# alexkeroro86/SampleNeRFRO

Measured on AMD Instinct MI355X. Metric: rays/sec (train step), higher is better.
Workload: dtype f16x3/fp32-acc

## Files before the change

include/rnerf.h:

```cpp
#ifndef RNERF_H_
#define RNERF_H_

#include <stddef.h>
#include <stdint.h>

#ifdef __cplusplus
extern "C" {
#endif

#define RNERF_VERSION 4

enum rnerf_status {
  RNERF_OK = 0,
  RNERF_ERR_ARG = -1,
  RNERF_ERR_HIP = -2,
  RNERF_ERR_UNSUPPORTED = -3
};

enum rnerf_precision {
  RNERF_PREC_F32 = 0,
  RNERF_PREC_F16X3 = 1,
  RNERF_PREC_BF16X3 = 2,
  RNERF_PREC_F16 = 3,
  RNERF_PREC_BF16 = 4,
// ... 29 lines not shown
const char* rnerf_last_error(void);
int rnerf_version(void);
int rnerf_device_cus(void);

int rnerf_grid_prefilter(const float* src, float* dst, float* tmp, const int32_t dims[3], int ksize, double ksigma,
                         void* stream);

int rnerf_grid_build_table(const float* grid, float* table, const rnerf_grid* g, void* stream);

int rnerf_grid_query(const float* table, const rnerf_grid* g, const float* pts, int64_t n, float* out, int32_t* idx,
                     void* stream);

int rnerf_march(const float* table, const rnerf_grid* g, const float* origins, const float* viewdirs, int32_t B,
                double near, double far, int32_t num_nodes, float* path_pd, float* path_dr, float* path_ior,
                int32_t* vox, void* stream);

size_t rnerf_nerfmlp_packed_bytes(int precision);
int rnerf_nerfmlp_pack(const float* params, int precision, void* packed, void* stream);

int rnerf_nerfmlp_forward(const void* packed, int precision, const float* rows_pd, const float* rows_dr,
                          const int32_t* node_of_sample, int32_t S, int32_t B, float* out_raw, int32_t max_workgroups, void* stream);

int rnerf_bkgd_forward(const float* params, const float* dirs, int32_t dir_stride, int64_t n, double rgb_padding,
                       float* out_rgb, void* stream);

int rnerf_composite(const float* raw, const float* rows_pd, const float* rows_dr, const int32_t* node_of_sample,
                    int32_t S, int32_t B, const float* bkgd, int white_bkgd, double rgb_padding, double sigma_bias,
                    float* rgb, float* dist, float* acc, float* trans, float* trans_bkgd, float* weights,
                    float* alpha, int mask_mode, const double* bbox, void* stream);

// ... 117 lines not shown
  int32_t randomized;
  int32_t use_random_choice;
  int32_t bg_patch_size;
  double bg_weight, bg_smooth_weight, annealed_alpha;
  double frozen_sq;
  int64_t frozen_count;
  void* aux_stream;
  void* grads_stream;
} rnerf_train_cfg;
typedef struct rnerf_prefetch {
  const float* origins;
  const float* viewdirs;
  float* path_pd;
  float* path_dr;
  void* side_stream;
} rnerf_prefetch;
size_t rnerf_train_workspace_bytes(const rnerf_model* m, const rnerf_train_cfg* c, int32_t B);
int rnerf_train_forward_backward(const rnerf_model* m, const rnerf_train_cfg* c, const float* theta, const float* origins, const float* viewdirs,
                                 const float* pixels, const float* env_dirs, int32_t B, const uint32_t* keys4, const int32_t* jitter_override,
                                 const float* u_override, int32_t u_per_ray, const float* path_pd, const float* path_dr, float* grads,
                                 void* workspace, int32_t max_workgroups, const rnerf_prefetch* next, void* stream);

#define RNERF_ADAM_SCRATCH_FLOATS 3076
typedef struct rnerf_adam_cfg {
  double lr_init, lr_final, lr_delay_mult;
  int64_t max_steps, lr_delay_steps;
  double b1, b2, eps;
  double weight_decay_mult, grad_max_val, grad_max_norm;
  int64_t n_all;
  double lr_override;
// ... 91 lines not shown
```

samplenerfro_amd/_lib.py:

```python
from __future__ import annotations

import ctypes as C
import os
from typing import Optional

HERE = os.path.dirname(os.path.abspath(__file__))
LIB_PATH = os.path.join(HERE, "lib", "librnerf.so")

PREC_F32, PREC_F16X3, PREC_BF16X3, PREC_F16, PREC_BF16, PREC_F16X2, PREC_F16F8 = 0, 1, 2, 3, 4, 5, 6
PRECISIONS = {"f32": PREC_F32, "f16x3": PREC_F16X3, "bf16x3": PREC_BF16X3, "f16": PREC_F16, "bf16": PREC_BF16, "f16x2": PREC_F16X2, "f16f8": PREC_F16F8}
BWD_BF16, BWD_F16, BWD_F16X2 = 0, 1, 2
BWD_F16X3 = BWD_F16X2
BWD_F16X3_LO8 = 4
BACKWARDS = {"f16x3": BWD_F16X3, "f16x3lo8": BWD_F16X3_LO8, "f16": BWD_F16, "bf16": BWD_BF16, "f32": BWD_F16X3, "tf32": BWD_F16}
BACKWARD_NAMES = {BWD_F16X3: "f16x3", BWD_F16X3_LO8: "f16x3lo8", BWD_F16: "f16", BWD_BF16: "bf16"}
TWO_PLANE_BACKWARDS = (BWD_F16X3, BWD_F16X3_LO8)
ABI_VERSION = 4
NERFMLP_PARAMS = 595844
BKGDMLP_PARAMS = 56963
SO3MLP_PARAMS = 65411
LPIPS_WEIGHT_FLOATS = 2470848


class RnerfError(RuntimeError):
# ... 25 lines not shown

class TrainCfg(C.Structure):
    _fields_ = [("backward", C.c_int32), ("randomized", C.c_int32), ("use_random_choice", C.c_int32), ("bg_patch_size", C.c_int32),
                ("bg_weight", C.c_double), ("bg_smooth_weight", C.c_double), ("annealed_alpha", C.c_double), ("frozen_sq", C.c_double),
                ("frozen_count", C.c_int64), ("aux_stream", C.c_void_p), ("grads_stream", C.c_void_p)]


class AdamCfg(C.Structure):
    _fields_ = [("lr_init", C.c_double), ("lr_final", C.c_double), ("lr_delay_mult", C.c_double), ("max_steps", C.c_int64),
                ("lr_delay_steps", C.c_int64), ("b1", C.c_double), ("b2", C.c_double), ("eps", C.c_double), ("weight_decay_mult", C.c_double),
                ("grad_max_val", C.c_double), ("grad_max_norm", C.c_double), ("n_all", C.c_int64), ("lr_override", C.c_double),
                ("use_lr_override", C.c_int32), ("skip_nonfinite", C.c_int32)]


class Prefetch(C.Structure):
    _fields_ = [("origins", C.c_void_p), ("viewdirs", C.c_void_p), ("path_pd", C.c_void_p), ("path_dr", C.c_void_p), ("side_stream", C.c_void_p)]


LEVEL_FLOATS = 9
ADAM_SCRATCH_FLOATS = 3076
_vp, _i32, _i64, _dbl = C.c_void_p, C.c_int32, C.c_int64, C.c_double
_GP = C.POINTER(Grid)
_MP, _TP, _AP = C.POINTER(Model), C.POINTER(TrainCfg), C.POINTER(AdamCfg)

SIGNATURES = {
    "rnerf_last_error": (C.c_char_p, []),
    "rnerf_version": (C.c_int, []),
    "rnerf_device_cus": (C.c_int, []),
    "rnerf_grid_prefilter": (C.c_int, [_vp, _vp, _vp, C.POINTER(_i32 * 3), C.c_int, _dbl, _vp]),
    "rnerf_grid_table_floats": (C.c_size_t, [_GP]),
    "rnerf_grid_build_table": (C.c_int, [_vp, _vp, _GP, _vp]),
    "rnerf_grid_query": (C.c_int, [_vp, _GP, _vp, _i64, _vp, _vp, _vp]),
    "rnerf_march": (C.c_int, [_vp, _GP, _vp, _vp, _i32, _dbl, _dbl, _i32, _vp, _vp, _vp, _vp, _vp]),
    "rnerf_nerfmlp_packed_bytes": (C.c_size_t, [C.c_int]),
    "rnerf_nerfmlp_pack": (C.c_int, [_vp, C.c_int, _vp, _vp]),
    "rnerf_nerfmlp_forward": (C.c_int, [_vp, C.c_int, _vp, _vp, _vp, _i32, _i32, _vp, _i32, _vp]),
    "rnerf_bkgd_forward": (C.c_int, [_vp, _vp, _i32, _i64, _dbl, _vp, _vp]),
    "rnerf_composite": (C.c_int, [_vp, _vp, _vp, _vp, _i32, _i32, _vp, C.c_int, _dbl, _dbl,
                                  _vp, _vp, _vp, _vp, _vp, _vp, _vp, C.c_int, C.POINTER(C.c_double * 6), _vp]),
    "rnerf_loss_reduce": (C.c_int, [_vp, _vp, _vp, _vp, _vp, _i32, _vp, _vp]),
    "rnerf_env_smooth_sum_floats": (C.c_size_t, [_i32]),
    "rnerf_env_smooth_backward": (C.c_int, [_vp, _i32, _dbl, _vp, _vp, _vp]),
    "rnerf_train_stats": (C.c_int, [_vp, _i32, _i32, _dbl, _vp, _i32, _dbl, _vp, _i64, _dbl, _i64, _vp, _vp]),
    "rnerf_composite_backward": (C.c_int, [_vp, _vp, _vp, _vp, _i32, _i32, _vp, _dbl, _dbl, _vp, _vp, _vp, _vp, _vp, _dbl, _dbl,
                                           _vp, _vp, C.c_int, C.c_int, C.c_int, C.POINTER(C.c_double * 6), _vp]),
    "rnerf_nerfmlp_save_bytes": (C.c_size_t, [_i64, C.c_int]),
    "rnerf_nerfmlp_dy_bytes": (C.c_size_t, [_i64, C.c_int]),
    "rnerf_nerfmlp_bwd_packed_bytes": (C.c_size_t, []),
# ... 120 lines not shown
```

samplenerfro_amd/csrc/march.hip:

```cpp
#include "common.h"

#include <stdlib.h>

namespace rnerf {

struct MarchParams {
  int dx, dy, dz;
  float nmin[3];
  double rcp_nd[3];
  unsigned sa[3], sb[3];
};

constexpr int kMarchAhead = 2;
constexpr int kMarchSets = kMarchAhead + 1;
constexpr int kMarchChunk = kMarchSets <= 4 ? 2 * kMarchSets : kMarchSets;
static_assert(2 * kMarchChunk * 512 <= 12 * 1024, "the ring must fit beside the weight-gradient kernel's LDS (148 KiB)");

__device__ __forceinline__ void march_chunk_barrier() { asm volatile("s_waitcnt lgkmcnt(0)\n\ts_barrier" ::: "memory"); }

template <bool WANT_IOR, bool WANT_VOX, bool BRICKS>
__global__ void __launch_bounds__(128) march_kernel(const float* __restrict__ table, MarchParams g,
                                                    const float* __restrict__ origins, const float* __restrict__ viewdirs,
                                                    int B, float near, float step, int num_nodes,
                                                    float* __restrict__ path_pd, float* __restrict__ path_dr,
                                                    float* __restrict__ path_ior, int* __restrict__ vox, int rays_per_wg) {
  constexpr int C = kMarchChunk;
  __shared__ float2 ring[2][C][64];
  const int lane = threadIdx.x & 63;
  const int wave = __builtin_amdgcn_readfirstlane((int)(threadIdx.x >> 6));
  const int q = lane & 3;
  int r = blockIdx.x * rays_per_wg + ((lane >> 2) & (rays_per_wg - 1));
  if (r >= B) r = B - 1;
  const int qc = q < 3 ? q : 0;
  const int nchunks = (num_nodes + C - 1) / C;
  const size_t node_stride = 4 * (size_t)B;

  if (wave != 0) {
    float* __restrict__ out_pd = path_pd + 4 * (size_t)r + q;
    float* __restrict__ out_dr = path_dr + 4 * (size_t)r + q;
    float rt = near, p_prev = 0.f;
    for (int c = 0; c < nchunks; ++c) {
      march_chunk_barrier();
      const float2* __restrict__ src = &ring[c & 1][0][lane];
#pragma unroll
      for (int s = 0; s < C; ++s) {
        const int k = c * C + s;
        if (k >= num_nodes) break;
        const float2 v = src[s * 64];
        const float p = v.x, d = v.y;
        if (k > 0) rt = fadd(rt, fsqrt(quad_sumsq3(fsub(p_prev, p))));
        p_prev = p;
        const float nrm = fsqrt(fmaxf(quad_sumsq3(d), 1e-6f));
        *out_pd = q < 3 ? p : rt;
        *out_dr = q < 3 ? fdiv(d, nrm) : 0.f;
        out_pd += node_stride; out_dr += node_stride;
      }
    }
    return;
  }

  const float nmin_q = g.nmin[qc];
  const double rcp_q = g.rcp_nd[qc];
  const int dim_q = qc == 0 ? g.dx : (qc == 1 ? g.dy : g.dz);
  const unsigned comp = (q + 1) & 3;
  const char* __restrict__ tabc = (const char*)table;
  const unsigned cofs = comp * 4u;
  const unsigned stride_q = g.sb[qc];
  const unsigned sa_q = g.sa[qc], sb_q = g.sb[qc];
  const int hi_q = dim_q - 1;
  float d = q < 3 ? viewdirs[3 * r + qc] : 0.f;
// ... 59 lines not shown
    d = fadd(d, fmul(step, c));
  };
  static_assert(C % kMarchSets == 0, "a chunk is a whole number of register rotations");
  for (int c = 0, k = 0; c < nchunks; ++c, k += C) {
    float2* slot = &ring[c & 1][0][lane];
#pragma unroll
    for (int u = 0; u < C; ++u) one_step(k + u, cs[u % kMarchSets], cs[(u + kMarchAhead) % kMarchSets], slot + 64 * u);
    march_chunk_barrier();
  }
}

}

using namespace rnerf;

extern "C" int rnerf_march(const float* table, const rnerf_grid* g, const float* origins, const float* viewdirs,
                           int32_t B, double near, double far, int32_t num_nodes, float* path_pd, float* path_dr,
                           float* path_ior, int32_t* vox, void* stream) {
  RNERF_CHECK_ARG(table && g && origins && viewdirs && path_pd && path_dr, "rnerf_march: null pointer");
  RNERF_CHECK_ARG(B > 0 && num_nodes >= 2, "rnerf_march: need B > 0 and num_nodes >= 2");
  RNERF_CHECK_ARG((((uintptr_t)table | (uintptr_t)path_pd | (uintptr_t)path_dr | (uintptr_t)path_ior) & 15) == 0,
                  "rnerf_march: table/path buffers must be 16-byte aligned");
  GridParams gp;
  RNERF_CHECK_ARG(make_grid_params(g, &gp), "rnerf_march: bad grid");
  RNERF_CHECK_ARG(grid_fits_march(gp), "rnerf_march: grid too large for 32-bit byte offsets (needs a table < 4 GiB and 24-bit strides: the row strides in reference order, the brick strides in bricks)");
  MarchParams p;
  p.dx = gp.dx; p.dy = gp.dy; p.dz = gp.dz;
  p.nmin[0] = gp.nminx; p.nmin[1] = gp.nminy; p.nmin[2] = gp.nminz;
  p.rcp_nd[0] = 1.0 / (double)gp.ndx; p.rcp_nd[1] = 1.0 / (double)gp.ndy; p.rcp_nd[2] = 1.0 / (double)gp.ndz;
  for (int i = 0; i < 3; ++i) { p.sa[i] = gp.sa[i]; p.sb[i] = gp.sb[i]; }
  const float stepf = (float)((far - near) / (num_nodes - 1));
  const float nearf = (float)near;
  const int rpw = 16;
  const dim3 block(128), grid((B + rpw - 1) / rpw);
  hipStream_t st = (hipStream_t)stream;
#define LAUNCH2(I, V, K)                                                                                           \
  hipLaunchKernelGGL((march_kernel<I, V, K>), grid, block, 0, st, table, p, origins, viewdirs, B, nearf, stepf, num_nodes, \
                     path_pd, path_dr, path_ior, vox, rpw)
#define LAUNCH(I, V) do { if (gp.layout == RNERF_TABLE_BRICKS) LAUNCH2(I, V, true); else LAUNCH2(I, V, false); } while (0)
  if (path_ior && vox) LAUNCH(true, true);
  else if (path_ior) LAUNCH(true, false);
  else if (vox) LAUNCH(false, true);
  else LAUNCH(false, false);
#undef LAUNCH
#undef LAUNCH2
  RNERF_CHECK_LAUNCH();
  return RNERF_OK;
}
```

samplenerfro_amd/csrc/pipeline.hip:

```cpp
#include "common.h"

#include <math.h>
#include <mutex>
#include <utility>
#include <vector>

namespace rnerf {
static int current_device_cus() {
  static int cache[64] = {0};
  int dev = 0;
  if (hipGetDevice(&dev) != hipSuccess || dev < 0 || dev >= 64) return 256;
  if (cache[dev] == 0) {
    int cus = 0;
    cache[dev] = (hipDeviceGetAttribute(&cus, hipDeviceAttributeMultiprocessorCount, dev) == hipSuccess && cus > 0) ? cus : 256;
  }
  return cache[dev];
}

namespace {
constexpr size_t kPoolCap = 32;
struct EventPool { std::vector<hipEvent_t> free_[64]; };
thread_local EventPool tl_pool;
inline hipError_t pool_get(hipEvent_t* e) {
  int dev = 0;
// ... 521 lines not shown
  if (aux) {
    RNERF_TRY(rnerf_fork(stream, aux));
    void* streams[2] = {t.packed_c, t.packed_f};
    void* dys[2] = {t.dy, t.dy_c};
    const int64_t dy_rows[2] = {(int64_t)(Nf > 0 ? S : Nc) * B, (int64_t)Nc * B};
    RNERF_TRY(nerfmlp_step_zero(prec, streams, Nf > 0 ? 2 : 1, bwd, dys, dy_rows, t.dy_c ? 2 : 1, (hipStream_t)aux));
    pre_zeroed = true;
    RNERF_TRY(nerfmlp_pack_impl(th_c, prec, t.packed_c, false, (hipStream_t)aux, false));
  }
  const int32_t* jitter = jitter_override;
  if (keys4) {
    RNERF_TRY(rnerf_rng_forward(keys4, Nc, m->num_path, c->use_random_choice, t.jitter, t.key_u, stream));
    if (!jitter_override) jitter = t.jitter;
  }
  if (!path_pd) {
    RNERF_TRY(rnerf_march(m->table, &m->grid, origins, viewdirs, B, m->near, m->far, N, f.path_pd, f.path_dr, nullptr, nullptr, stream));
    path_pd = f.path_pd; path_dr = f.path_dr;
  }
  hipLaunchKernelGGL(bkgd_dirs_kernel, dim3((B + M + 255) / 256), dim3(256), 0, st, (const float4*)path_dr, jitter, Nc, B, env_dirs, M, (float4*)f.bk_dirs);
  RNERF_CHECK_LAUNCH();
  RNERF_TRY(rnerf_bkgd_forward_train(th_b, f.bk_dirs, 4, (int64_t)B + M, m->rgb_padding, t.out_all, t.save_bk, stream));
  const float* bkgd = t.out_all;
  const float* rgb_env = t.out_all + (size_t)3 * B;
  if (aux) {
    RNERF_TRY(rnerf_join(stream, aux));
    if (Nf > 0) {
      RNERF_TRY(nerfmlp_pack_impl(th_f, prec, t.packed_f, false, (hipStream_t)aux, false));
      RNERF_TRY(mark_point((hipStream_t)aux, &fine_packed.e));
    }
    RNERF_CHECK_HIP(hipMemsetAsync(grads, 0, (size_t)(n_theta + 8) * sizeof(float), (hipStream_t)aux));
    RNERF_TRY(rnerf_nerfmlp_pack_bwd(th_c, bwd, t.packed_bwd, aux));
// ... 15 lines not shown
    if (!aux) RNERF_TRY(rnerf_nerfmlp_pack(th_f, prec, t.packed_f, stream));
    else { hipEvent_t e = fine_packed.e; fine_packed.e = nullptr; RNERF_TRY(wait_point(st, e)); }
    RNERF_TRY(rnerf_nerfmlp_forward_train(t.packed_f, prec, f.rows_pd, f.rows_dr, nullptr, S, B, f.raw_f, t.save_f, bwd, max_workgroups, stream));
    lf = level_of(t.level_f, B);
    RNERF_TRY(rnerf_composite(f.raw_f, f.rows_pd, f.rows_dr, nullptr, S, B, bkgd, m->white_bkgd, m->rgb_padding, m->sigma_bias, lf.rgb, lf.dist, lf.acc, lf.trans,
                              lf.tb, nullptr, nullptr, level_mask_mode(m), level_mask_box(m), stream));
    if (m->bd_cut == 1) RNERF_TRY(bd_cut_pair(m, f.raw_f, f.rows_pd, f.rows_dr, S, B, bkgd, lf, f.tmp_level, f.tmp_level2, stream));
  }
  RNERF_TRY(rnerf_loss_reduce(Nf > 0 ? lc.rgb : nullptr, lf.rgb, lf.trans, lf.tb, pixels, B, t.sums, stream));
  const double bg_on = (c->bg_weight > 0 && c->annealed_alpha > 0) ? 1.0 : 0.0;
  const double mse_scale = 2.0 / (3.0 * B);
  const double env_on = c->annealed_alpha > 0 ? 1.0 : 0.0;
  if (!aux) RNERF_CHECK_HIP(hipMemsetAsync(grads, 0, (size_t)(n_theta + 8) * sizeof(float), st));
  auto march_next = [&]() -> int {
    RNERF_CHECK_ARG(next->origins && next->viewdirs && next->path_pd && next->path_dr && next->side_stream, "rnerf_train_forward_backward: incomplete rnerf_prefetch");
    RNERF_TRY(rnerf_fork(stream, next->side_stream));
    return rnerf_march(m->table, &m->grid, next->origins, next->viewdirs, B, m->near, m->far, N, next->path_pd, next->path_dr, nullptr, nullptr,
                       next->side_stream);
  };
  if (aux) RNERF_TRY(rnerf_join(stream, aux));
  float* d_first = t.d_all;
  const bool split_levels = levels_side_by_side(m, c, B);
  float* d_raw_c = split_levels ? t.d_raw_c : t.d_raw;
  void* dy_c = split_levels ? t.dy_c : t.dy;
  if (Nf > 0) {
    RNERF_TRY(rnerf_composite_backward(f.raw_f, f.rows_pd, f.rows_dr, nullptr, S, B, bkgd, m->rgb_padding, m->sigma_bias, lf.rgb, pixels, lf.trans, lf.tb, t.sums,
                                       mse_scale, c->bg_weight * bg_on, t.d_raw, d_first, 0, m->white_bkgd, m->bd_cut == 1 ? 1 : level_mask_mode(m), m->bd_cut ? m->bd_cut_bbox : nullptr, stream));
    if (split_levels) {
      RNERF_TRY(rnerf_composite_backward(f.raw_c, path_pd, path_dr, jitter, Nc, B, bkgd, m->rgb_padding, m->sigma_bias, lc.rgb, pixels, nullptr, nullptr, nullptr,
                                         mse_scale, 0.0, d_raw_c, d_first, 1, m->white_bkgd, level_mask_mode(m), level_mask_box(m), stream));
      RNERF_TRY(rnerf_fork(stream, aux));
      if (smooth) RNERF_TRY(rnerf_env_smooth_backward(rgb_env, ps, c->bg_smooth_weight * env_on, t.d_all + (size_t)3 * B, t.env_sum, aux));
      RNERF_TRY(rnerf_bkgd_backward(th_b, t.save_bk, t.d_all, (int64_t)B + M, m->rgb_padding, t.dy_bk, g_b, nullptr, aux));
// ... 181 lines not shown
```

samplenerfro_amd/models.py:

```python
from __future__ import annotations

import ctypes as C
import math
import os
import weakref
from typing import Any, Dict, List, Optional, Sequence, Tuple

import numpy as np
import torch

from . import _lib, ops, prng
from ._lib import Grid, PRECISIONS
from .utils import Rays

NERF_MLP_SHAPES = [(63, 256), (256, 256), (256, 256), (256, 256), (256, 256), (319, 256), (256, 256), (256, 256),
                   (256, 1), (256, 256), (283, 128), (128, 3)]
BKGD_MLP_SHAPES = [(27, 128), (128, 128), (128, 128), (155, 128), (128, 3)]
SO3_MLP_SHAPES = [(60, 128), (128, 128), (128, 128), (188, 128), (128, 3)]


_STREAMS: Dict[Tuple[str, str], "torch.cuda.Stream"] = {}


def shared_stream(device, role: str) -> "torch.cuda.Stream":
# ... 197 lines not shown
            raise NotImplementedError("prefetch_path: the all* march depends on the so3_mlp parameters; call apply() without a handle")
        if self._side is None:
            self._side = shared_stream(self.device, "march")
        self._mlp_wg_limit = max(_lib.load().rnerf_device_cus() - int(reserve_cus), 1) if reserve_cus > 0 else 0
        cur = torch.cuda.current_stream()
        if sync_inputs:
            self._side.wait_stream(cur)
        with torch.cuda.stream(self._side):
            rays.origins.record_stream(self._side); rays.viewdirs.record_stream(self._side)
            pd, dr, ior, _ = ops.march(self.table, self.spec, rays.origins, rays.viewdirs, self.near, self.far,
                                       self.num_samples, want_ior=self.use_online_sparsity)
            ev = torch.cuda.Event()
            ev.record(self._side)
        return PathHandle(pd, dr, ior, ev, rays.origins.shape[0])

    def prefetch_slot(self, rays: Rays):
        if not self.stage.startswith("radiance"):
            raise NotImplementedError("prefetch: the all* march depends on the so3_mlp parameters")
        if self._side is None:
            self._side = shared_stream(self.device, "march")
        o, v = ops._chk(rays.origins, "origins"), ops._chk(rays.viewdirs, "viewdirs")
        B = o.shape[0]
        pd = torch.empty((self.num_samples, B, 4), dtype=torch.float32, device=self.device)
        dr = torch.empty_like(pd)
        for t in (o, v, pd, dr):
            t.record_stream(self._side)
        h = PathHandle(pd, dr, None, torch.cuda.Event(), B)
        h.keep = (o, v)
        return h, _lib.Prefetch(o.data_ptr(), v.data_ptr(), pd.data_ptr(), dr.data_ptr(), self._side.cuda_stream)

    def tail_stream(self) -> torch.cuda.Stream:
        if getattr(self, "_tail", None) is None:
            self._tail = shared_stream(self.device, "tail")
        return self._tail

    def comm_stream(self) -> torch.cuda.Stream:
        return self.tail_stream()

    def release_reserved_cus(self) -> None:
        self._mlp_wg_limit = 0

    def c_model(self, variables=None, precision: Optional[int] = None) -> "_lib.Model":
        prec = self.precision if precision is None else int(precision)
        m = _lib.Model()
# ... 56 lines not shown
        if Nf > 0:
            if u_fine is not None:
                u = ops._chk(u_fine, "u_fine"); per_ray = 1 if u.dim() == 2 else 0
            elif not randomized:
                u = self.make_u(None, B, False)
            else:
                if jitter is not None:
                    key, _ = prng.split(np.asarray(rng_1, np.uint32))
                    u = self.make_u(key, B, True)
                else:
                    u = torch.empty((Nf, B), dtype=torch.float32, device=self.device)
                    _lib.check(lib.rnerf_stratified_u_dev(key_u.data_ptr(), B, Nf, u.data_ptr(), st), "rnerf_stratified_u_dev")
                per_ray = 1
        pd = dr = None
        if path is not None:
            if path.batch != B:
                raise ValueError("path handle was marched for a different batch size")
            cur = torch.cuda.current_stream()
            cur.wait_event(path.event)
            pd, dr = path.pd, path.dr
            pd.record_stream(cur); dr.record_stream(cur)
        ws = self._workspace("fwd", lib.rnerf_forward_workspace_bytes(C.byref(m), B))
        out_c = torch.empty(_lib.LEVEL_FLOATS * B, dtype=torch.float32, device=self.device)
        out_f = torch.empty(_lib.LEVEL_FLOATS * B, dtype=torch.float32, device=self.device) if Nf > 0 else None
        _lib.check(lib.rnerf_forward(C.byref(m), o.data_ptr(), v.data_ptr(), B, jit.data_ptr(), _lib.ptr(u), per_ray, _lib.ptr(pd), _lib.ptr(dr),
                                     out_c.data_ptr(), _lib.ptr(out_f), ws.data_ptr(), int(self._mlp_wg_limit), st), "rnerf_forward")
        return [level_views(t, B) for t in (out_c, out_f) if t is not None]

    def apply(self, variables, *args, method=None, **kwargs):
        if method is not None:
# ... 4 lines not shown
                jitter=None, u_fine: Optional[torch.Tensor] = None, taps: Optional[dict] = None,
                path: Optional["PathHandle"] = None, ctx: Optional[dict] = None,
                noise_c: Optional[torch.Tensor] = None, noise_f: Optional[torch.Tensor] = None):
        origins, viewdirs = rays.origins, rays.viewdirs
        if origins.dim() != 2 or origins.shape[-1] != 3:
            raise ValueError("rays.origins must be [B, 3]")
        B = origins.shape[0]
        noisy = self.noise_std is not None and randomized
        if ctx is None and taps is None and self.whole_path and self.stage.startswith("radiance") and not self.use_online_sparsity and not noisy:
            return self._forward_whole(variables, rng_0, rng_1, rays, randomized, jitter, u_fine, path), 0.0
        Nc, Nf, N = self.num_coarse_samples, self.num_fine_samples, self.num_samples
        key, rng_0 = prng.split(np.asarray(rng_0, np.uint32))
        sparsity = self.use_online_sparsity and (ctx is None or (bool(ctx.get("loss_sp")) and not self.stage.startswith("all")))
        want_ior = sparsity or (taps is not None and not (ctx is not None and self.stage.startswith("all")))
        if path is not None:
            if path.batch != B:
                raise ValueError("path handle was marched for a different batch size")
            cur = torch.cuda.current_stream()
            cur.wait_event(path.event)
            path_pd, path_dr, path_ior = path.pd, path.dr, path.ior
            for t in (path_pd, path_dr, path_ior):
                if t is not None:
                    t.record_stream(cur)
            if want_ior and path_ior is None:
                raise ValueError("path handle lacks the IoR record (prefetch it from a model with the same options)")
        elif self.stage.startswith("all") and ctx is not None:
            rec = ops.march_all_train(self.table, self.spec, self._flat(variables, "so3_mlp", SO3_MLP_SHAPES).detach(), origins, viewdirs,
                                      self.near, self.far, N, annealed_alpha, lazy=True)
            ctx["march_rec"] = rec
            path_pd, path_dr, path_ior = rec["path_pd"], rec["path_dr"], None
# ... 142 lines not shown
        loss_sp = (alpha - coarse_alpha_target).abs().mean()
        next_c, next_f = alpha.mean(), 0.0
        if self.num_fine_samples > 0 and self.use_fine_sparsity:
            alpha = alpha_of("fine_mlp", self.fine_step_size)
            loss_sp = loss_sp + (alpha - fine_alpha_target).abs().mean()
            next_f = alpha.mean()
        return loss_sp, next_c, next_f


def level_views(out: torch.Tensor, B: int):
    return (out[:3 * B].view(B, 3), out[3 * B:4 * B], out[4 * B:5 * B], out[5 * B:6 * B].view(B, 1), out[6 * B:9 * B].view(B, 3))


class PathHandle:

    def __init__(self, pd, dr, ior, event, batch):
        self.pd, self.dr, self.ior, self.event, self.batch = pd, dr, ior, event, batch


def make_variables(flat: Dict[str, torch.Tensor]) -> Dict[str, Any]:
    params: Dict[str, Any] = {"coarse_mlp": flat_to_tree(flat["coarse_mlp"], NERF_MLP_SHAPES),
                              "bkgd_mlp": flat_to_tree(flat["bkgd_mlp"], BKGD_MLP_SHAPES)}
    if "fine_mlp" in flat:
        params["fine_mlp"] = flat_to_tree(flat["fine_mlp"], NERF_MLP_SHAPES)
    if "so3_mlp" in flat:
        params["path_sampler"] = {"scan": {"idx_model": {"so3_mlp": flat_to_tree(flat["so3_mlp"], SO3_MLP_SHAPES)}}}
    return {"params": params, "flat": dict(flat)}


def construct_nerf(key, example_batch, args, ndim, nmin, nmax, grid, precision: str = "f16x3", device=None, eval_precision: Optional[str] = None):
    if args.rgb_activation != "sigmoid" or args.sigma_activation != "softplus" or args.net_activation != "relu":
        raise NotImplementedError("the HIP kernels implement relu / sigmoid / softplus (the reference defaults, rnerf/utils.py:168-175)")
# ... 17 lines not shown
```

samplenerfro_amd/ops.py:

```python
from __future__ import annotations

import ctypes as C
import os
import weakref
from typing import Optional, Tuple

import torch

from . import _lib
from ._lib import Grid, check, current_stream, ptr


def _chk(t: torch.Tensor, name: str, dtype=torch.float32) -> torch.Tensor:
    if not t.is_cuda:
        raise _lib.RnerfError(f"{name}: expected a CUDA (ROCm) tensor; the hot path has no CPU implementation")
    if t.dtype != dtype:
        raise _lib.RnerfError(f"{name}: expected dtype {dtype}, got {t.dtype}")
    return t if t.is_contiguous() else t.contiguous()


_workspaces: dict = {}


def workspace(name: str, *args, device, keep_for: Optional[int] = None) -> torch.Tensor:
# ... 81 lines not shown
def march(table: torch.Tensor, spec: Grid, origins: torch.Tensor, viewdirs: torch.Tensor, near: float, far: float,
          num_nodes: int, want_ior: bool = False, want_vox: bool = False, out=None):
    lib = _lib.load()
    table = _chk(table, "table"); o = _chk(origins, "origins"); d = _chk(viewdirs, "viewdirs")
    B = o.shape[0]
    if out is not None:
        path_pd, path_dr = out
    else:
        path_pd = torch.empty((num_nodes, B, 4), dtype=torch.float32, device=o.device)
        path_dr = torch.empty((num_nodes, B, 4), dtype=torch.float32, device=o.device)
    ior = torch.empty((num_nodes, B, 4), dtype=torch.float32, device=o.device) if want_ior else None
    vox = torch.empty((num_nodes, B, 6), dtype=torch.int32, device=o.device) if want_vox else None
    check(lib.rnerf_march(ptr(table), C.byref(spec), ptr(o), ptr(d), B, float(near), float(far), int(num_nodes),
                          ptr(path_pd), ptr(path_dr), ptr(ior), ptr(vox), current_stream()), "rnerf_march")
    return path_pd, path_dr, ior, vox


def nerfmlp_pack(params_flat: torch.Tensor, precision: int, out: Optional[torch.Tensor] = None) -> torch.Tensor:
    lib = _lib.load()
    p = _chk(params_flat, "params_flat")
    if p.numel() != _lib.NERFMLP_PARAMS:
        raise _lib.RnerfError(f"NerfMLP flat params must have {_lib.NERFMLP_PARAMS} floats, got {p.numel()}")
    nbytes = lib.rnerf_nerfmlp_packed_bytes(int(precision))
    if nbytes == 0:
        check(-1, "rnerf_nerfmlp_packed_bytes")
    if out is None:
        out = torch.empty(nbytes, dtype=torch.uint8, device=p.device)
    check(lib.rnerf_nerfmlp_pack(ptr(p), int(precision), ptr(out), current_stream()), "rnerf_nerfmlp_pack")
    return out

# ... 681 lines not shown
```

samplenerfro_amd/prng.py:

```python
from __future__ import annotations

import numpy as np

_ROT = ((13, 15, 26, 6), (17, 29, 16, 24))


def _rotl(x, r):
    return ((x << np.uint32(r)) | (x >> np.uint32(32 - r))).astype(np.uint32)


def threefry2x32(k0, k1, x0, x1):
    with np.errstate(over="ignore"):
        k0 = np.uint32(k0); k1 = np.uint32(k1)
        ks = (k0, k1, np.uint32(k0 ^ k1 ^ np.uint32(0x1BD11BDA)))
        x0 = (np.asarray(x0, np.uint32) + ks[0]).astype(np.uint32)
        x1 = (np.asarray(x1, np.uint32) + ks[1]).astype(np.uint32)
        for i in range(5):
            for r in _ROT[i % 2]:
                x0 = (x0 + x1).astype(np.uint32)
                x1 = _rotl(x1, r)
                x1 = (x1 ^ x0).astype(np.uint32)
            x0 = (x0 + ks[(i + 1) % 3]).astype(np.uint32)
            x1 = (x1 + ks[(i + 2) % 3] + np.uint32(i + 1)).astype(np.uint32)
    return x0, x1
# ... 25 lines not shown


def randint(key, shape, minval: int, maxval: int) -> np.ndarray:
    k1, k2 = split(key)
    hi = random_bits(k1, shape).astype(np.uint64)
    lo = random_bits(k2, shape).astype(np.uint64)
    span = np.uint64(max(int(maxval) - int(minval), 1))
    m32 = np.uint64(0xFFFFFFFF)
    mult = (np.uint64(2 ** 16) % span)
    mult = ((mult * mult) & m32) % span
    off = (((hi % span) * mult) & m32) + (lo % span)
    off = (off & m32) % span
    return (np.int64(minval) + off.astype(np.int64)).astype(np.int32)


_ERFINV_CENTRAL = (2.81022636e-08, 3.43273939e-07, -3.5233877e-06, -4.39150654e-06, 0.00021858087, -0.00125372503, -0.00417768164,
                   0.246640727, 1.50140941)
_ERFINV_TAIL = (-0.000200214257, 0.000100950558, 0.00134934322, -0.00367342844, 0.00573950773, -0.0076224613, 0.00943887047,
                1.00167406, 2.83297682)


def erf_inv_f32(x: np.ndarray) -> np.ndarray:
    f = np.float32
    x = np.asarray(x, f)
    edge = np.abs(x) == f(1.0)
    w = (-np.log1p(-(np.where(edge, f(0), x) ** 2).astype(f))).astype(f)
    central = w < f(5.0)
    wc = (w - f(2.5)).astype(f)
    wt = (np.sqrt(np.maximum(w, f(0))).astype(f) - f(3.0)).astype(f)

# ... 22 lines not shown
```

samplenerfro_amd/train.py:

```python
from __future__ import annotations

import contextlib
import ctypes as C
import os
import weakref
from typing import Any, Dict, Optional

import numpy as np
import torch

from . import _lib, distributed, ops, prng
from .models import BKGD_MLP_SHAPES, NERF_MLP_SHAPES, SO3_MLP_SHAPES, NerfModel, make_variables
from .utils import Rays, Stats, learning_rate_decay

_RANGE_RETRY_LAG = 2
_LAG_SLOTS = 8
_SKIP_NONFINITE_UPDATES = True

_N_STATS = 8


class TrainState:

    def __init__(self, step, theta, mu, nu, variables, segments, lr_fn, flags=None):
# ... 219 lines not shown
    state.sync_step_counter()
    fs = frozen_sq_of(state, state.variables)
    frozen = state.variables["flat"].get("so3_mlp") if fs[1] > 0 else None
    word = getattr(state, "_lag_word", None)
    _lib.check(lib.rnerf_adam_update_fused(C.byref(a), state.theta.data_ptr(), state.mu.data_ptr(), state.nu.data_ptr(), state.grads.data_ptr(),
                                           state.theta.numel(), _lib.ptr(frozen), fs[1], state.step_dev.data_ptr(), state.adam_scratch.data_ptr(),
                                           word, _lib.current_stream()), "rnerf_adam_update_fused")
    if word is not None:
        state._lag_word_written = True
    state.step += 1
    state._step_dev_value = state.step
    state._staged_bad = None
    _bump(state.theta)


def _train_step_whole(model: NerfModel, rng, state: TrainState, batch, flags, jitter, u_fine, path, next_rays):
    lib = _lib.load()
    rng, key_0, key_1 = prng.split(np.asarray(rng, np.uint32), 3)
    annealed = float(np.asarray(batch["annealed_alpha"]).reshape(-1)[0])
    rays: Rays = batch["rays"]
    o, v = ops._chk(rays.origins, "origins"), ops._chk(rays.viewdirs, "viewdirs")
    pixels = ops._chk(batch["pixels"][..., :3].contiguous(), "pixels")
    B = o.shape[0]
    env = None
    if flags.bg_smooth_weight > 0:
        env = ops._chk(batch["env_rays"].viewdirs.reshape(-1, 3), "env_rays.viewdirs")
        if env.shape[0] != flags.bg_patch_size ** 2:
            raise ValueError("env_rays.viewdirs must hold bg_patch_size^2 directions")
    m = model.c_model()
    c = train_cfg(model, state, flags, annealed)
    st = _lib.current_stream()
    keys = model._keys_dev(key_0, key_1)
    jit = model._jitter_dev(jitter) if jitter is not None else None
    u, per_ray = None, 0
    if u_fine is not None:
        u = ops._chk(u_fine, "u_fine"); per_ray = 1 if u.dim() == 2 else 0
    pd = dr = None
    if path is not None:
        if path.batch != B:
            raise ValueError("path handle was marched for a different batch size")
        cur = torch.cuda.current_stream()
        cur.wait_event(path.event)
        pd, dr = path.pd, path.dr
        pd.record_stream(cur); dr.record_stream(cur)
    ws = model._workspace("train", lib.rnerf_train_workspace_bytes(C.byref(m), C.byref(c), B))
    G = state.grads
    n_theta = state.theta.numel()
    nxt, next_path = None, None
    if next_rays is not None:
        next_path, nxt = model.prefetch_slot(next_rays)
    comm = model.comm_stream() if (distributed.active() and hasattr(model, "comm_stream")) else None
    if comm is not None:
        c = _lib.TrainCfg.from_buffer_copy(c)
        c.grads_stream = comm.cuda_stream
    _lib.check(lib.rnerf_train_forward_backward(C.byref(m), C.byref(c), state.theta.data_ptr(), o.data_ptr(), v.data_ptr(), pixels.data_ptr(), _lib.ptr(env), B,
                                                keys.data_ptr(), _lib.ptr(jit), _lib.ptr(u), per_ray, _lib.ptr(pd), _lib.ptr(dr), G.data_ptr(), ws.data_ptr(),
                                                int(model._mlp_wg_limit), C.byref(nxt) if nxt is not None else None, st), "rnerf_train_forward_backward")
    if next_path is not None:
        next_path.event.record(model._side)
    if comm is not None:
        n_big = state.segments["bkgd_mlp"][0]
        with torch.cuda.stream(comm):
            pending = distributed.allreduce_begin(G[:n_big])
        distributed.allreduce_mean_([G[n_big:]])
        distributed.allreduce_end_mean_(pending, G[:n_big])
# ... 164 lines not shown
                     noise_c=None, noise_f=None, _guard: bool = False):
    flags = state.flags if flags is None else flags
    all_stage = flags.stage.startswith("all")
    if flags.stage.startswith("ior"):
        return _ior_stage_step(model, rng, state, batch, flags)
    if not (flags.stage.startswith("radiance") or all_stage):
        raise NotImplementedError(f"train_step: unknown stage {flags.stage!r}")
    if all_stage and model.stage != flags.stage:
        raise ValueError("stage all*: build the model with the same stage (the march must evaluate so3_mlp)")
    if flags.beta_weight > 0 or flags.sparsity_weight > 0:
        pass
    noisy = getattr(model, "noise_std", None) is not None and bool(flags.randomized)
    if not all_stage and taps is None and forward_taps is None and getattr(model, "whole_path", False) and not noisy:
        return _train_step_whole(model, rng, state, batch, flags, jitter, u_fine, path, next_rays)
    rng, key_0, key_1 = prng.split(np.asarray(rng, np.uint32), 3)
    annealed = float(np.asarray(batch["annealed_alpha"]).reshape(-1)[0])
    rays: Rays = batch["rays"]
    pixels = batch["pixels"][..., :3].contiguous()
    variables = state.variables
    prec = model.precision
    if all_stage and next_rays is not None:
        if model._side is None:
            from .models import shared_stream
            model._side = shared_stream(model.device, "march")
        ops.prefetch_shell_order(model.table, model.spec, next_rays.origins, next_rays.viewdirs, model.near, model.far, model.num_samples, model._side)
        next_rays = None
    Nc, Nf = model.num_coarse_samples, model.num_fine_samples
    bwd = backward_mode(flags, model)
    if all_stage and bwd == _lib.BWD_BF16:
        raise ValueError('stage all*: the input gradients are built on the row-normalised backward modes (backward_precision "f16x3" or "f16")')
# ... 107 lines not shown
```

Before: 685,000.

## March only the jittered sample nodes for flat models, precomputing next-step keys

For flat models (no fine samples), the ray march now writes path records only at the node each coarse sample's jitter selects, and skips the normalisation and stores for every other node. The prefetch for the next step pre-splits the RNG keys on the host and generates the jitter on the side stream before marching, so the sparse march is ready when that step runs. The goal is to cut the march's global memory writes by roughly a factor of num_path. It adds a lazily densified PathHandle and guards that fall back to a full march whenever keys don't match or a dense path is required.

```diff
diff --git a/include/rnerf.h b/include/rnerf.h
--- a/include/rnerf.h
+++ b/include/rnerf.h
@@ -67,6 +67,9 @@
 int rnerf_march(const float* table, const rnerf_grid* g, const float* origins, const float* viewdirs, int32_t B,
                 double near, double far, int32_t num_nodes, float* path_pd, float* path_dr, float* path_ior,
                 int32_t* vox, void* stream);
+int rnerf_march_sparse(const float* table, const rnerf_grid* g, const float* origins, const float* viewdirs, int32_t B,
+                       double near, double far, int32_t num_nodes, float* path_pd, float* path_dr,
+                       const int32_t* sample_nodes, int32_t num_path, void* stream);
 
 size_t rnerf_nerfmlp_packed_bytes(int precision);
 int rnerf_nerfmlp_pack(const float* params, int precision, void* packed, void* stream);
@@ -214,6 +217,8 @@
   float* path_pd;
   float* path_dr;
   void* side_stream;
+  const uint32_t* next_keys4;
+  int32_t* sample_nodes;
 } rnerf_prefetch;
 size_t rnerf_train_workspace_bytes(const rnerf_model* m, const rnerf_train_cfg* c, int32_t B);
 int rnerf_train_forward_backward(const rnerf_model* m, const rnerf_train_cfg* c, const float* theta, const float* origins, const float* viewdirs,
diff --git a/samplenerfro_amd/_lib.py b/samplenerfro_amd/_lib.py
--- a/samplenerfro_amd/_lib.py
+++ b/samplenerfro_amd/_lib.py
@@ -63,7 +63,8 @@
 
 
 class Prefetch(C.Structure):
-    _fields_ = [("origins", C.c_void_p), ("viewdirs", C.c_void_p), ("path_pd", C.c_void_p), ("path_dr", C.c_void_p), ("side_stream", C.c_void_p)]
+    _fields_ = [("origins", C.c_void_p), ("viewdirs", C.c_void_p), ("path_pd", C.c_void_p), ("path_dr", C.c_void_p), ("side_stream", C.c_void_p),
+                ("next_keys4", C.c_void_p), ("sample_nodes", C.c_void_p)]
 
 
 LEVEL_FLOATS = 9
@@ -81,6 +82,7 @@
     "rnerf_grid_build_table": (C.c_int, [_vp, _vp, _GP, _vp]),
     "rnerf_grid_query": (C.c_int, [_vp, _GP, _vp, _i64, _vp, _vp, _vp]),
     "rnerf_march": (C.c_int, [_vp, _GP, _vp, _vp, _i32, _dbl, _dbl, _i32, _vp, _vp, _vp, _vp, _vp]),
+    "rnerf_march_sparse": (C.c_int, [_vp, _GP, _vp, _vp, _i32, _dbl, _dbl, _i32, _vp, _vp, _vp, _i32, _vp]),
     "rnerf_nerfmlp_packed_bytes": (C.c_size_t, [C.c_int]),
     "rnerf_nerfmlp_pack": (C.c_int, [_vp, C.c_int, _vp, _vp]),
     "rnerf_nerfmlp_forward": (C.c_int, [_vp, C.c_int, _vp, _vp, _vp, _i32, _i32, _vp, _i32, _vp]),
diff --git a/samplenerfro_amd/csrc/march.hip b/samplenerfro_amd/csrc/march.hip
--- a/samplenerfro_amd/csrc/march.hip
+++ b/samplenerfro_amd/csrc/march.hip
@@ -18,12 +18,13 @@
 
 __device__ __forceinline__ void march_chunk_barrier() { asm volatile("s_waitcnt lgkmcnt(0)\n\ts_barrier" ::: "memory"); }
 
-template <bool WANT_IOR, bool WANT_VOX, bool BRICKS>
+template <bool WANT_IOR, bool WANT_VOX, bool BRICKS, bool SPARSE>
 __global__ void __launch_bounds__(128) march_kernel(const float* __restrict__ table, MarchParams g,
                                                     const float* __restrict__ origins, const float* __restrict__ viewdirs,
                                                     int B, float near, float step, int num_nodes,
                                                     float* __restrict__ path_pd, float* __restrict__ path_dr,
-                                                    float* __restrict__ path_ior, int* __restrict__ vox, int rays_per_wg) {
+                                                    float* __restrict__ path_ior, int* __restrict__ vox, int rays_per_wg,
+                                                    const int* __restrict__ sample_nodes, int num_path) {
   constexpr int C = kMarchChunk;
   __shared__ float2 ring[2][C][64];
   const int lane = threadIdx.x & 63;
@@ -39,6 +40,8 @@
     float* __restrict__ out_pd = path_pd + 4 * (size_t)r + q;
     float* __restrict__ out_dr = path_dr + 4 * (size_t)r + q;
     float rt = near, p_prev = 0.f;
+    int group = 0, left = num_path, wanted = 0;
+    if constexpr (SPARSE) wanted = sample_nodes[0];
     for (int c = 0; c < nchunks; ++c) {
       march_chunk_barrier();
       const float2* __restrict__ src = &ring[c & 1][0][lane];
@@ -50,10 +53,18 @@
         const float p = v.x, d = v.y;
         if (k > 0) rt = fadd(rt, fsqrt(quad_sumsq3(fsub(p_prev, p))));
         p_prev = p;
-        const float nrm = fsqrt(fmaxf(quad_sumsq3(d), 1e-6f));
-        *out_pd = q < 3 ? p : rt;
-        *out_dr = q < 3 ? fdiv(d, nrm) : 0.f;
+        if (!SPARSE || k == wanted) {
+          const float nrm = fsqrt(fmaxf(quad_sumsq3(d), 1e-6f));
+          *out_pd = q < 3 ? p : rt;
+          *out_dr = q < 3 ? fdiv(d, nrm) : 0.f;
+        }
         out_pd += node_stride; out_dr += node_stride;
+        if constexpr (SPARSE) {
+          if (--left == 0) {
+            left = num_path; ++group;
+            wanted = (group + 1) * num_path <= num_nodes ? sample_nodes[group] : -1;
+          }
+        }
       }
     }
     return;
@@ -143,9 +154,9 @@
 
 using namespace rnerf;
 
-extern "C" int rnerf_march(const float* table, const rnerf_grid* g, const float* origins, const float* viewdirs,
-                           int32_t B, double near, double far, int32_t num_nodes, float* path_pd, float* path_dr,
-                           float* path_ior, int32_t* vox, void* stream) {
+static int march_impl(const float* table, const rnerf_grid* g, const float* origins, const float* viewdirs,
+                      int32_t B, double near, double far, int32_t num_nodes, float* path_pd, float* path_dr,
+                      float* path_ior, int32_t* vox, const int32_t* sample_nodes, int32_t num_path, void* stream) {
   RNERF_CHECK_ARG(table && g && origins && viewdirs && path_pd && path_dr, "rnerf_march: null pointer");
   RNERF_CHECK_ARG(B > 0 && num_nodes >= 2, "rnerf_march: need B > 0 and num_nodes >= 2");
   RNERF_CHECK_ARG((((uintptr_t)table | (uintptr_t)path_pd | (uintptr_t)path_dr | (uintptr_t)path_ior) & 15) == 0,
@@ -164,10 +175,17 @@
   const dim3 block(128), grid((B + rpw - 1) / rpw);
   hipStream_t st = (hipStream_t)stream;
 #define LAUNCH2(I, V, K)                                                                                           \
-  hipLaunchKernelGGL((march_kernel<I, V, K>), grid, block, 0, st, table, p, origins, viewdirs, B, nearf, stepf, num_nodes, \
-                     path_pd, path_dr, path_ior, vox, rpw)
+  hipLaunchKernelGGL((march_kernel<I, V, K, false>), grid, block, 0, st, table, p, origins, viewdirs, B, nearf, stepf, num_nodes, \
+                     path_pd, path_dr, path_ior, vox, rpw, (const int*)nullptr, 0)
 #define LAUNCH(I, V) do { if (gp.layout == RNERF_TABLE_BRICKS) LAUNCH2(I, V, true); else LAUNCH2(I, V, false); } while (0)
-  if (path_ior && vox) LAUNCH(true, true);
+  if (sample_nodes) {
+    if (gp.layout == RNERF_TABLE_BRICKS)
+      hipLaunchKernelGGL((march_kernel<false, false, true, true>), grid, block, 0, st, table, p, origins, viewdirs, B, nearf, stepf, num_nodes,
+                         path_pd, path_dr, path_ior, vox, rpw, sample_nodes, num_path);
+    else
+      hipLaunchKernelGGL((march_kernel<false, false, false, true>), grid, block, 0, st, table, p, origins, viewdirs, B, nearf, stepf, num_nodes,
+                         path_pd, path_dr, path_ior, vox, rpw, sample_nodes, num_path);
+  } else if (path_ior && vox) LAUNCH(true, true);
   else if (path_ior) LAUNCH(true, false);
   else if (vox) LAUNCH(false, true);
   else LAUNCH(false, false);
@@ -176,3 +194,17 @@
   RNERF_CHECK_LAUNCH();
   return RNERF_OK;
 }
+
+extern "C" int rnerf_march(const float* table, const rnerf_grid* g, const float* origins, const float* viewdirs,
+                           int32_t B, double near, double far, int32_t num_nodes, float* path_pd, float* path_dr,
+                           float* path_ior, int32_t* vox, void* stream) {
+  return march_impl(table, g, origins, viewdirs, B, near, far, num_nodes, path_pd, path_dr, path_ior, vox, nullptr, 0, stream);
+}
+
+extern "C" int rnerf_march_sparse(const float* table, const rnerf_grid* g, const float* origins, const float* viewdirs,
+                                  int32_t B, double near, double far, int32_t num_nodes, float* path_pd, float* path_dr,
+                                  const int32_t* sample_nodes, int32_t num_path, void* stream) {
+  RNERF_CHECK_ARG(!sample_nodes || (num_path >= 1 && num_nodes % num_path == 0),
+                  "rnerf_march_sparse: sample_nodes needs num_path >= 1 and num_nodes a multiple of num_path");
+  return march_impl(table, g, origins, viewdirs, B, near, far, num_nodes, path_pd, path_dr, nullptr, nullptr, sample_nodes, num_path, stream);
+}
diff --git a/samplenerfro_amd/csrc/pipeline.hip b/samplenerfro_amd/csrc/pipeline.hip
--- a/samplenerfro_amd/csrc/pipeline.hip
+++ b/samplenerfro_amd/csrc/pipeline.hip
@@ -559,7 +559,8 @@
     if (!jitter_override) jitter = t.jitter;
   }
   if (!path_pd) {
-    RNERF_TRY(rnerf_march(m->table, &m->grid, origins, viewdirs, B, m->near, m->far, N, f.path_pd, f.path_dr, nullptr, nullptr, stream));
+    const int32_t* sampled = (Nf == 0 && keys4 && !jitter_override) ? t.jitter : nullptr;
+    RNERF_TRY(rnerf_march_sparse(m->table, &m->grid, origins, viewdirs, B, m->near, m->far, N, f.path_pd, f.path_dr, sampled, m->num_path, stream));
     path_pd = f.path_pd; path_dr = f.path_dr;
   }
   hipLaunchKernelGGL(bkgd_dirs_kernel, dim3((B + M + 255) / 256), dim3(256), 0, st, (const float4*)path_dr, jitter, Nc, B, env_dirs, M, (float4*)f.bk_dirs);
@@ -605,9 +606,13 @@
   if (!aux) RNERF_CHECK_HIP(hipMemsetAsync(grads, 0, (size_t)(n_theta + 8) * sizeof(float), st));
   auto march_next = [&]() -> int {
     RNERF_CHECK_ARG(next->origins && next->viewdirs && next->path_pd && next->path_dr && next->side_stream, "rnerf_train_forward_backward: incomplete rnerf_prefetch");
+    RNERF_CHECK_ARG((next->next_keys4 == nullptr) == (next->sample_nodes == nullptr), "rnerf_train_forward_backward: rnerf_prefetch needs both next_keys4 and sample_nodes or neither");
+    RNERF_CHECK_ARG(!next->sample_nodes || Nf == 0, "rnerf_train_forward_backward: rnerf_prefetch.sample_nodes is for flat models (num_fine == 0) only");
     RNERF_TRY(rnerf_fork(stream, next->side_stream));
-    return rnerf_march(m->table, &m->grid, next->origins, next->viewdirs, B, m->near, m->far, N, next->path_pd, next->path_dr, nullptr, nullptr,
-                       next->side_stream);
+    if (next->sample_nodes)
+      RNERF_TRY(rnerf_rng_forward(next->next_keys4, Nc, m->num_path, c->use_random_choice, next->sample_nodes, nullptr, next->side_stream));
+    return rnerf_march_sparse(m->table, &m->grid, next->origins, next->viewdirs, B, m->near, m->far, N, next->path_pd, next->path_dr,
+                              next->sample_nodes, m->num_path, next->side_stream);
   };
   if (aux) RNERF_TRY(rnerf_join(stream, aux));
   float* d_first = t.d_all;
diff --git a/samplenerfro_amd/models.py b/samplenerfro_amd/models.py
--- a/samplenerfro_amd/models.py
+++ b/samplenerfro_amd/models.py
@@ -235,7 +235,7 @@
             ev.record(self._side)
         return PathHandle(pd, dr, ior, ev, rays.origins.shape[0])
 
-    def prefetch_slot(self, rays: Rays):
+    def prefetch_slot(self, rays: Rays, next_keys=None):
         if not self.stage.startswith("radiance"):
             raise NotImplementedError("prefetch: the all* march depends on the so3_mlp parameters")
         if self._side is None:
@@ -248,7 +248,18 @@
             t.record_stream(self._side)
         h = PathHandle(pd, dr, None, torch.cuda.Event(), B)
         h.keep = (o, v)
-        return h, _lib.Prefetch(o.data_ptr(), v.data_ptr(), pd.data_ptr(), dr.data_ptr(), self._side.cuda_stream)
+        nxt = _lib.Prefetch(o.data_ptr(), v.data_ptr(), pd.data_ptr(), dr.data_ptr(), self._side.cuda_stream)
+        if next_keys is not None:
+            if self.num_fine_samples > 0:
+                raise ValueError("prefetch_slot: a hierarchical model resamples arbitrary nodes and needs every record (next_keys=None)")
+            keys = self._keys_dev(*next_keys)
+            jit = torch.empty(self.num_coarse_samples, dtype=torch.int32, device=self.device)
+            keys.record_stream(self._side); jit.record_stream(self._side)
+            h.sparse, h.jitter, h.key = True, jit, np.array(next_keys[0], np.uint32).reshape(2).copy()
+            h.keep = (o, v, keys)
+            h._march_args = (self.table, self.spec, self.near, self.far, self.num_samples)
+            nxt.next_keys4, nxt.sample_nodes = keys.data_ptr(), jit.data_ptr()
+        return h, nxt
 
     def tail_stream(self) -> torch.cuda.Stream:
         if getattr(self, "_tail", None) is None:
@@ -335,6 +346,7 @@
                 per_ray = 1
         pd = dr = None
         if path is not None:
+            path.need_dense("NerfModel.apply")
             if path.batch != B:
                 raise ValueError("path handle was marched for a different batch size")
             cur = torch.cuda.current_stream()
@@ -369,6 +381,7 @@
         sparsity = self.use_online_sparsity and (ctx is None or (bool(ctx.get("loss_sp")) and not self.stage.startswith("all")))
         want_ior = sparsity or (taps is not None and not (ctx is not None and self.stage.startswith("all")))
         if path is not None:
+            path.need_dense("NerfModel.apply")
             if path.batch != B:
                 raise ValueError("path handle was marched for a different batch size")
             cur = torch.cuda.current_stream()
@@ -541,8 +554,47 @@
 
 class PathHandle:
 
-    def __init__(self, pd, dr, ior, event, batch):
-        self.pd, self.dr, self.ior, self.event, self.batch = pd, dr, ior, event, batch
+    def __init__(self, pd, dr, ior, event, batch, sparse=False, jitter=None, key=None):
+        self._pd, self._dr, self.ior, self.event, self.batch = pd, dr, ior, event, batch
+        self.sparse, self.jitter, self.key = bool(sparse), jitter, key
+        self._march_args = None
+
+    def raw(self):
+        return self._pd, self._dr
+
+    @property
+    def pd(self):
+        self.complete()
+        return self._pd
+
+    @property
+    def dr(self):
+        self.complete()
+        return self._dr
+
+    def complete(self) -> None:
+        if not self.sparse:
+            return
+        if self._march_args is None:
+            raise ValueError("this sparse path handle does not know its rays: it cannot be completed")
+        table, spec, near, far, N = self._march_args
+        cur = torch.cuda.current_stream()
+        cur.wait_event(self.event)
+        pd, dr, _, _ = ops.march(table, spec, self.keep[0], self.keep[1], near, far, N)
+        rest = torch.ones(N, dtype=torch.bool, device=pd.device)
+        rest[self.jitter.long()] = False
+        self._pd[rest] = pd[rest]
+        self._dr[rest] = dr[rest]
+        self._pd.record_stream(cur); self._dr.record_stream(cur)
+        self.sparse = False
+
+    def need_dense(self, who: str) -> None:
+        if self.sparse:
+            raise ValueError(f"{who}: this path handle holds the records of its own jitter's nodes only (a flat train step's prefetch); "
+                             "march the rays with prefetch_path() or pass path=None")
+
+    def matches(self, key_0) -> bool:
+        return self.key is not None and np.array_equal(np.asarray(self.key, np.uint32).reshape(-1), np.asarray(key_0, np.uint32).reshape(-1))
 
 
 def make_variables(flat: Dict[str, torch.Tensor]) -> Dict[str, Any]:
diff --git a/samplenerfro_amd/ops.py b/samplenerfro_amd/ops.py
--- a/samplenerfro_amd/ops.py
+++ b/samplenerfro_amd/ops.py
@@ -119,6 +119,22 @@
     check(lib.rnerf_march(ptr(table), C.byref(spec), ptr(o), ptr(d), B, float(near), float(far), int(num_nodes),
                           ptr(path_pd), ptr(path_dr), ptr(ior), ptr(vox), current_stream()), "rnerf_march")
     return path_pd, path_dr, ior, vox
+
+
+def march_sparse(table: torch.Tensor, spec: Grid, origins: torch.Tensor, viewdirs: torch.Tensor, near: float, far: float,
+                 num_nodes: int, sample_nodes: Optional[torch.Tensor], num_path: int, out):
+    lib = _lib.load()
+    table = _chk(table, "table"); o = _chk(origins, "origins"); d = _chk(viewdirs, "viewdirs")
+    path_pd, path_dr = out
+    B = o.shape[0]
+    if any(tuple(t.shape) != (num_nodes, B, 4) or not t.is_contiguous() for t in (path_pd, path_dr)):
+        raise ValueError("march_sparse: out must be two contiguous [num_nodes, B, 4] float32 tensors")
+    _chk(path_pd, "path_pd"); _chk(path_dr, "path_dr")
+    if sample_nodes is not None and (sample_nodes.dtype != torch.int32 or not sample_nodes.is_contiguous() or sample_nodes.numel() * int(num_path) != num_nodes):
+        raise ValueError("march_sparse: sample_nodes must be contiguous int32 [num_nodes // num_path]")
+    check(lib.rnerf_march_sparse(ptr(table), C.byref(spec), ptr(o), ptr(d), B, float(near), float(far), int(num_nodes),
+                                 ptr(path_pd), ptr(path_dr), ptr(sample_nodes), int(num_path), current_stream()), "rnerf_march_sparse")
+    return path_pd, path_dr
 
 
 def nerfmlp_pack(params_flat: torch.Tensor, precision: int, out: Optional[torch.Tensor] = None) -> torch.Tensor:
diff --git a/samplenerfro_amd/prng.py b/samplenerfro_amd/prng.py
--- a/samplenerfro_amd/prng.py
+++ b/samplenerfro_amd/prng.py
@@ -63,6 +63,19 @@
     return (np.int64(minval) + off.astype(np.int64)).astype(np.int32)
 
 
+def step_keys(rng):
+    out = split(np.asarray(rng, np.uint32), 3)
+    return out[0], out[1], out[2]
+
+
+def step_jitter(key_0, num_coarse: int, num_path: int, use_random_choice: bool) -> np.ndarray:
+    key, _ = split(np.asarray(key_0, np.uint32))
+    j = np.arange(0, num_coarse * num_path, num_path, dtype=np.int32)
+    if use_random_choice:
+        j = j + randint(key, (num_coarse,), 0, num_path)
+    return j.astype(np.int32)
+
+
 _ERFINV_CENTRAL = (2.81022636e-08, 3.43273939e-07, -3.5233877e-06, -4.39150654e-06, 0.00021858087, -0.00125372503, -0.00417768164,
                    0.246640727, 1.50140941)
 _ERFINV_TAIL = (-0.000200214257, 0.000100950558, 0.00134934322, -0.00367342844, 0.00573950773, -0.0076224613, 0.00943887047,
diff --git a/samplenerfro_amd/train.py b/samplenerfro_amd/train.py
--- a/samplenerfro_amd/train.py
+++ b/samplenerfro_amd/train.py
@@ -257,9 +257,20 @@
     _bump(state.theta)
 
 
+def _split3(state: TrainState, rng, ahead: bool = False):
+    r = np.asarray(rng, np.uint32)
+    held = getattr(state, "_split_ahead", None)
+    if held is not None and np.array_equal(held[0], r):
+        return held[1]
+    out = prng.step_keys(r)
+    if ahead:
+        state._split_ahead = (r.copy(), out)
+    return out
+
+
 def _train_step_whole(model: NerfModel, rng, state: TrainState, batch, flags, jitter, u_fine, path, next_rays):
     lib = _lib.load()
-    rng, key_0, key_1 = prng.split(np.asarray(rng, np.uint32), 3)
+    rng, key_0, key_1 = _split3(state, rng)
     annealed = float(np.asarray(batch["annealed_alpha"]).reshape(-1)[0])
     rays: Rays = batch["rays"]
     o, v = ops._chk(rays.origins, "origins"), ops._chk(rays.viewdirs, "viewdirs")
@@ -279,19 +290,25 @@
     if u_fine is not None:
         u = ops._chk(u_fine, "u_fine"); per_ray = 1 if u.dim() == 2 else 0
     pd = dr = None
+    flat = model.num_fine_samples == 0
+    if path is not None and path.sparse and not (flat and jit is None and path.matches(key_0)):
+        path = None
     if path is not None:
         if path.batch != B:
             raise ValueError("path handle was marched for a different batch size")
         cur = torch.cuda.current_stream()
         cur.wait_event(path.event)
-        pd, dr = path.pd, path.dr
+        pd, dr = path.raw()
         pd.record_stream(cur); dr.record_stream(cur)
+        if path.sparse:
+            jit = path.jitter
+            jit.record_stream(cur)
     ws = model._workspace("train", lib.rnerf_train_workspace_bytes(C.byref(m), C.byref(c), B))
     G = state.grads
     n_theta = state.theta.numel()
     nxt, next_path = None, None
     if next_rays is not None:
-        next_path, nxt = model.prefetch_slot(next_rays)
+        next_path, nxt = model.prefetch_slot(next_rays, next_keys=_split3(state, rng, ahead=True)[1:] if flat else None)
     comm = model.comm_stream() if (distributed.active() and hasattr(model, "comm_stream")) else None
     if comm is not None:
         c = _lib.TrainCfg.from_buffer_copy(c)
@@ -486,6 +503,8 @@
     if not all_stage and taps is None and forward_taps is None and getattr(model, "whole_path", False) and not noisy:
         return _train_step_whole(model, rng, state, batch, flags, jitter, u_fine, path, next_rays)
     rng, key_0, key_1 = prng.split(np.asarray(rng, np.uint32), 3)
+    if path is not None and path.sparse:
+        path = None
     annealed = float(np.asarray(batch["annealed_alpha"]).reshape(-1)[0])
     rays: Rays = batch["rays"]
     pixels = batch["pixels"][..., :3].contiguous()
```

New measurement: 694,200 (median of 6 runs). 1.01x the previous value.
